# kjyv/FloBaRoID

Measured on AMD Instinct MI355X. Metric: regressor samples/s (fused regressor->Gram pass) + TSQR TFLOP/s, WALK-MAN 31-DOF float-base, higher is better.
Workload: dtype f64

## Files before the change

### flobaroid_amd/csrc/fbr_gram64.h

```cpp
#pragma once
#define FBR_G64_SWZ(c) (2 * ((c) & 15))
#include <algorithm>
#include <type_traits>
#include <utility>

#include "fbr_kinid.h"

struct FbrGram64Tile {
    int col[FBR_TILE];
    std::vector<int> path;
    int friction = 0;
    int lo = 0, hi = 0;
};

struct FbrGram64 {
    int NT = 0;
    int NF = 0;
    int nlev = 0, fb = 0, flev = 0, ntr = 0, maxact = 0, npw = 0, wpb = 8;
    long blk_doubles = 0;
    std::vector<int> trow;
    std::vector<int> slab;
    int nstage = 0, base_stages = 0;
    std::vector<int> stage_lev;
    std::vector<int> lev_begin;
// ... 356 lines not shown
                                    int tiling = 1)
{
    if (gp.T != 1 || (gp.k > 0 && gp.rhs_tiles)) return false;
    std::vector<FbrGram64Tile> prog;
    if (!fbr_gram64_program_tiles(hm, gp, prog)) return false;
    std::vector<int> pairs;
    for (size_t s = 0; s < gp.slots.size(); s++) {
        const int pi = gp.slots[s].pair;
        if (pi < 0) continue;
        if (gp.pairs[pi].mode != 0) return false;
        pairs.insert(pairs.end(), {gp.pairs[pi].I, gp.pairs[pi].J});
    }
    bool ok = fbr_gram64_build_tiles(hm, gp.cfg, prog, pairs, g, force_tiles, wide16) && fbr_gram64_lds_bytes(g) <= FBR_G64_LDS_MAX;
    g.tiling = 0;
    if (!ok || !tiling) return ok;
    std::vector<FbrGram64Tile> fill;
    fbr_gram64_fill_tiles(hm, prog, fill);
    FbrGram64 c;
    if (fbr_gram64_build_tiles(hm, gp.cfg, fill, {}, c, force_tiles, wide16) && fbr_gram64_lds_bytes(c) <= FBR_G64_LDS_MAX &&
        (c.mfma_per_block < g.mfma_per_block || (c.mfma_per_block == g.mfma_per_block && c.ntr < g.ntr))) {
        g = std::move(c);
        g.tiling = 1;
    }
    return true;
}

#define FBR_G64_WORDS 18
#define FBR_G64_FRIC 4
struct FbrGram64Producer {
    int nparts = 1, nslots = 1, step0[FBR_KINWRITE_PARTS] = {0, 0, 0, 0}, nsteps[FBR_KINWRITE_PARTS] = {0, 0, 0, 0};
    std::vector<long long> rel;
    std::vector<int> lcol;
    std::vector<int> steps;
};

static inline bool fbr_gram64_build_producer(const FbrHostModel &hm, const FbrGram64 &g, FbrGram64Producer &pr)
{
    std::vector<int> tile_of(hm.cols, -1), slot_of(hm.cols, -1);
    for (int t = 0; t < g.NT; t++)
        for (int sl = 0; sl < FBR_TILE; sl++)
            if (g.tiles[t].col[sl] >= 0 && g.tiles[t].col[sl] < hm.cols) {
                tile_of[g.tiles[t].col[sl]] = t;
                slot_of[g.tiles[t].col[sl]] = sl;
            }
    std::vector<double> lcost(hm.L, 30.0);
    for (int c = 0; c < hm.ninert; c++)
        if (tile_of[c] >= 0) lcost[hm.coldesc[c].link] += 10.0 + (double)(hm.fb + hm.path[hm.coldesc[c].link].size());
    std::vector<FbrKinIdProgram> progs;
    std::vector<std::vector<char>> own;
    try {
        fbr_kinid_build_parts(hm, lcost, FBR_KINWRITE_PARTS, progs, own);
    } catch (const std::exception &) {
        return false;
    }
    pr.nparts = (int)progs.size();
    pr.rel.assign((size_t)pr.nparts * FBR_G64_WORDS * hm.L, 0);
    pr.lcol.assign((size_t)pr.nparts * (10 + FBR_G64_FRIC) * hm.L, -1);
    const int nfric = hm.n > 0 ? (hm.cols - hm.ninert) / hm.n : 0;
    if (nfric > FBR_G64_FRIC) return false;
    auto word = [](long long tile_row, int sl) { return ((tile_row * 1024 + sl * 32) * 8) | (long long)FBR_G64_SWZ(sl) | (1LL << 62); };
    for (int c = 0; c < hm.ninert; c++) {
        const int t = tile_of[c], sl = slot_of[c], l = hm.coldesc[c].link, pidx = hm.coldesc[c].pidx;
        if (t < 0) continue;
        if (!FbrGramProgram::nested(g.tiles[t].path, hm.path[l]) || hm.path[l].size() > g.tiles[t].path.size()) return false;
        const long long tr0 = (long long)g.trow[(size_t)t * g.nlev + g.tile_lo[t]] - g.tile_lo[t];
        if (tr0 < 0) return false;
        for (int pq = 0; pq < pr.nparts; pq++)
            if (own[pq][l]) {
                long long *w14 = &pr.rel[((size_t)pq * hm.L + l) * FBR_G64_WORDS];
                w14[pidx] = word(tr0, sl);
                if (g.fcol_tile[c] >= 0) {
                    if (pidx >= 4) return false;
                    w14[10 + pidx] = word(g.trow[(size_t)g.fcol_tile[c] * g.nlev], g.fcol_slot[c]);
                }
                pr.lcol[((size_t)pq * hm.L + l) * 10 + pidx] = c;
            }
    }
    for (int c = hm.ninert; c < hm.cols; c++) {
        const int t = tile_of[c], sl = slot_of[c], d = hm.coldesc[c].joint, p = (c - hm.ninert) / std::max(hm.n, 1);
        if (t < 0) continue;
        int l = -1;
        for (int x = 0; x < hm.L; x++)
            if (hm.dof[x] == d) l = x;
        if (l < 0 || p >= FBR_G64_FRIC || hm.path[l].empty() || hm.path[l].back() != d) return false;
        const int lv = hm.fb + (int)hm.path[l].size() - 1;
        if (lv < g.tile_lo[t] || g.trow[(size_t)t * g.nlev + lv] < 0) return false;
        const long long tr0 = (long long)g.trow[(size_t)t * g.nlev + g.tile_lo[t]] - g.tile_lo[t];
        if (tr0 < 0) return false;
        for (int pq = 0; pq < pr.nparts; pq++)
            if (own[pq][l]) {
                pr.rel[((size_t)pq * hm.L + l) * FBR_G64_WORDS + 14 + p] = word(tr0, sl);
                pr.lcol[(size_t)pr.nparts * 10 * hm.L + ((size_t)pq * hm.L + l) * FBR_G64_FRIC + p] = c;
            }
    }
    pr.steps.clear();
    pr.nslots = 1;
    for (int pq = 0; pq < pr.nparts; pq++) {
        pr.step0[pq] = (int)(pr.steps.size() / FBR_KINID_STEP);
        pr.nsteps[pq] = progs[pq].nsteps;
        pr.nslots = std::max(pr.nslots, progs[pq].nslots);
        pr.steps.insert(pr.steps.end(), progs[pq].steps.begin(), progs[pq].steps.begin() + (size_t)progs[pq].nsteps * FBR_KINID_STEP);
    }
    return true;
}

static inline bool fbr_gram64_build_producer(const FbrHostModel &hm, const FbrGramProgram &, const FbrGram64 &g, FbrGram64Producer &pr)
{
    return fbr_gram64_build_producer(hm, g, pr);
}

#define FBR_G64_MAXK 2
#include "fbr_mom_lanes.h"
FBR_HD int fbr_gram64_mom_count(int cols, int k) { return k * cols + k * (k + 1) / 2; }
FBR_HD void fbr_gram64_mom_target(int cols, int k, int idx, int *row, int *col)
{
    if (idx < k * cols) {
        *row = idx % cols;
        *col = cols + idx / cols;
        return;
    }
    int e = idx - k * cols, i = 0;
    while (e >= k - i) e -= k - i, i++;
    *row = cols + i;
    *col = cols + i + e;
}

#define FBR_G64_LANECOL_RHS 24
static inline std::vector<int> fbr_gram64_lane_columns(const FbrGram64Producer &pr, int L)
{
    std::vector<int> t((size_t)pr.nparts * L * 64, -1);
    for (int pq = 0; pq < pr.nparts; pq++)
        for (int l = 0; l < L; l++)
            for (int r = 0; r < FBR_G64_MAXK; r++) {
                int *row = &t[((size_t)pq * L + l) * 64];
                for (int p = 0; p < 10; p++) {
                    const int c = pr.lcol[((size_t)pq * L + l) * 10 + p];
// ... 122 lines not shown
        const int ls = min(lane, valid - 1);
        const long s = base + ls;
        const bool live = lane < valid;
        const double *mysq = sq + ls * ldn, *mysdq = sdq + ls * ldn, *mysddq = sddq + ls * ldn, *myw = sw + ls * ldw, *myt = st + ls * ldw;
        const long slot_off = blk * blk_doubles + (long)(lane >> 5) * 512;
        const int s31 = lane & 31;
        auto state = [&](int d, double &a, double &b, double &c) {
            a = mysq[d];
            b = mysdq[d];
            c = mysddq[d];
        };
        auto basest = [&](double *v6, double *a6, double *e3) {
            for (int i = 0; i < 6; i++) {
                v6[i] = bv[s * 6 + i];
                a6[i] = ba[s * 6 + i];
            }
            for (int i = 0; i < 3; i++) e3[i] = rpy[s * 3 + i];
        };
        auto save = [&](int b, int i, double v) { scr[(b * FBR_LINK_REC + i) * 64] = v; };
        auto load = [&](int b, int i) { return scr[(b * FBR_LINK_REC + i) * 64]; };
        auto consts = [&](int l, double *rR, double *rp, double *ax) {
            const fbr_cdouble_ptr cR = (fbr_cdouble_ptr)(unsigned long)m.restR, cp = (fbr_cdouble_ptr)(unsigned long)m.restp,
                                  ca = (fbr_cdouble_ptr)(unsigned long)m.axis;
            for (int i = 0; i < 9; i++) rR[i] = cR[9 * l + i];
            for (int i = 0; i < 3; i++) {
                rp[i] = cp[3 * l + i];
                ax[i] = ca[3 * l + i];
            }
        };
        const unsigned vlane = (unsigned)(((unsigned long)slot_off + (unsigned long)s31) << 3);
        auto link = [&](int l, int depth, const double *rec, const double (*Sst)[6], const int *lvd, double *F) {
            (void)F;
            if (wr.base_only) depth = 0;
            int mycol = -1;
            if (domom) mycol = glcol[l * 64];
            __builtin_amdgcn_s_waitcnt(0x0F70);
            double macc = 0.0;
            auto mom_sum = [&](auto g0c, auto ngc, auto p0c, auto nqc, const double *v, int r) {
                constexpr int G0 = decltype(g0c)::value, NG = decltype(ngc)::value, P0 = decltype(p0c)::value, NQ = decltype(nqc)::value;
                double u[NG];
#pragma unroll
                for (int i = 0; i < NG; i++) u[i] = (G0 + i >= P0 && G0 + i < P0 + NQ) ? v[G0 + i - P0] : 0.0;
                const double sum = fbr_mom_lanes_sum<NG>(u, live, mx);
                if (G0 == 0 ? (lane & 15) == 6 * r : (lane & 7) == 1 + 6 * r) macc += sum;
            };
            long d10[10], dF[4];
#pragma unroll
            for (int pp = 0; pp < 10; pp++) d10[pp] = cdst[((long)part * m.L + l) * FBR_G64_WORDS + pp];
#pragma unroll
            for (int pp = 0; pp < 4; pp++) dF[pp] = cdst[((long)part * m.L + l) * FBR_G64_WORDS + 10 + pp];
            auto ft_of = [&](int ro, double *F) {
#pragma unroll
                for (int i = 0; i < 6; i++)
                    if (i < m.fb) F[i] = myt[ro + i];
#pragma unroll
                for (int j = 0; j < MAXD; j++)
                    if (j < depth) {
                        const double tj = myt[ro + m.fb + lvd[j]];
#pragma unroll
                        for (int i = 0; i < 6; i++) F[i] += Sst[j][i] * tj;
                    }
            };
            double Ft[6] = {0.0, 0.0, 0.0, 0.0, 0.0, 0.0};
            if constexpr (KR == 1) {
                if (wr.k) {
#pragma unroll
// ... 422 lines not shown
```

### flobaroid_amd/csrc/fbr_gram_api.hip

```cpp
#define FBR_KERNELS_GRAM
#include "fbr_internal.h"

static int get_deal(GramHolder *h, int wpg, GramHolder::Deal *out, bool base_only = false)
{
    const int key = wpg | (base_only ? 1 << 24 : 0);
    auto it = h->deals.find(key);
    if (it != h->deals.end()) {
        *out = it->second;
        return FBR_OK;
    }
    const std::vector<int> n = fbr_gram_deal(h->prog, wpg, base_only);
    std::vector<int2> tab;
    std::vector<int> begin(h->prog.T + 1, 0), given(h->prog.T, 0);
    for (int p = 0; p < h->prog.T; p++) begin[p + 1] = begin[p] + n[p];
    while ((int)tab.size() < begin[h->prog.T])
        for (int p = 0; p < h->prog.T; p++)
            if (given[p] < n[p]) tab.push_back(make_int2(p, given[p]++ | (n[p] << 16)));
    GramHolder::Deal d;
    int rc;
    if ((rc = upload(h->pool, tab, &d.tab))) return rc;
    if ((rc = upload(h->pool, begin, &d.begin))) return rc;
    h->deals[key] = d;
    *out = d;
    return FBR_OK;
// ... 227 lines not shown
{
    const int Pa = m->hm.cols + k;
    const size_t cnt = (size_t)Pa * Pa;
    int rc;
    if ((rc = m->gram_r_tmp.ensure(cnt * sizeof(double)))) return rc;
    double *R = m->gram_r_tmp.as<double>();
    if ((rc = tsqr_impl(m, st, nullptr, 0, rhs, k, w, nullptr, R, FBR_DEVICE, nullptr))) return rc;
    double *G = G_out;
    if (out_mem == FBR_HOST) {
        if ((rc = m->g_tmp.ensure(cnt * sizeof(double)))) return rc;
        G = m->g_tmp.as<double>();
        if (accumulate) HIPCHK(hipMemcpyAsync(G, G_out, cnt * sizeof(double), hipMemcpyHostToDevice, m->stream));
    }
    hipLaunchKernelGGL(fbr_rtr_kernel, dim3(1024), dim3(256), 0, m->stream, Pa, R, G, accumulate ? 1 : 0);
    HIPCHK(hipGetLastError());
    return finish_output(m, G, G_out, cnt, out_mem);
}
static size_t gram64_plds(const FbrHostModel &hm, int k, bool has_w)
{
    return ((size_t)3 * 64 * (std::max(hm.n, 1) | 1) + (size_t)((has_w ? 1 : 0) + k) * 64 * (hm.rows | 1)) * sizeof(double);
}

static int get_gram64(fbr_model *m, GramHolder *h)
{
    if (h->g64_state) return FBR_OK;
    h->g64_state = -1;
    const FbrHostModel &hm = m->hm;
    if (m->kinid.nsteps <= 0 || !fbr_gram64_build(hm, h->prog, h->g64, m->opt.gram_force_tiles != 0, m->opt.gram_lane_waves >= 16,
                                                         (int)m->opt.gram_lane_tiling))
        return FBR_OK;
    FbrGram64 &g = h->g64;
    if (fbr_gram64_lds_bytes(g) > FBR_G64_LDS_MAX) return FBR_OK;
    if (gram64_plds(hm, h->prog.k, true) > 160 * 1024) return FBR_OK;
    if (!fbr_gram64_build_producer(hm, g, h->g64p)) return FBR_OK;
    std::vector<int> wgbegin{0, 0};
    int rc;
    if ((rc = upload(h->pool, g.slab, &h->d64_slab)) || (rc = upload(h->pool, g.lev_begin, &h->d64_levb)) || (rc = upload(h->pool, g.pieces, &h->d64_pieces)) ||
        (rc = upload(h->pool, g.wmeta, &h->d64_wmeta)) || (rc = upload(h->pool, h->g64p.lcol, &h->d64_lcol)) ||
        (rc = upload(h->pool, fbr_gram64_lane_columns(h->g64p, hm.L), &h->d64_lanecol)) ||
        (rc = upload(h->pool, h->g64p.steps, &h->d64_steps)) ||
        (rc = upload(h->pool, g.slot_tiles, &h->d64_slot_tiles)) || (rc = upload(h->pool, g.tilecol, &h->d64_tilecol)) ||
        (rc = upload(h->pool, g.stage_lev, &h->d64_stagelev)) || (!g.runs.empty() && (rc = upload(h->pool, g.runs, &h->d64_runs))))
        return rc;
    h->g64_state = 1;
    return FBR_OK;
}

static int gram64_serves(fbr_model *m, GramHolder *h, int k, bool *serves)
{
    *serves = false;
    if (!m->opt.gram_lane || k > FBR_G64_MAXK || (k > 0 && !h->moments)) return FBR_OK;
    if (int rc = get_gram64(m, h)) return rc;
    *serves = h->g64_state == 1;
    return FBR_OK;
}

static long gram64_chunk_blocks(const FbrGram64 &g) { return std::max<long>(1, (long)((size_t)3 * 1024 * 1024 * 1024 / ((size_t)g.blk_doubles * 8))); }

static int gram64_wg_table(GramHolder *h, int wgs, const int **out)
{
    auto it = h->d64_wb.find(wgs);
    if (it == h->d64_wb.end()) {
        std::vector<int> wb{0, wgs};
        const int *dwb = nullptr;
        if (int rc = upload(h->pool, wb, &dwb)) return rc;
        it = h->d64_wb.emplace(wgs, dwb).first;
    }
    *out = it->second;
    return FBR_OK;
}

static int gram64_ensure_images(fbr_model *m, GramHolder *h, long chb)
{
// ... 27 lines not shown
static int gram64_setup(fbr_model *m, GramHolder *h, bool base_only, Gram64Launch *L)
{
    const FbrGram64 &g = h->g64;
    L->kp = kinid_params(m, 0, h->g64p.nslots, h->d64_steps);
    L->pgrid_max = kinimg_by_depth(m, [](auto D) { return D <= 10 ? 2 : 1; }) * m->num_cus;
    if (int rc = h->scr64.ensure((size_t)L->pgrid_max * h->g64p.nparts * std::max(h->g64p.nslots, 1) * FBR_LINK_REC * 64 * sizeof(double))) return rc;
    DevGram64 &dg = L->dg;
    dg.NT = g.NT + g.NF;
    dg.nlev = g.nlev;
    dg.maxact = g.maxact;
    dg.npieces = (int)g.pieces.size() / 2;
    dg.blk_doubles = g.blk_doubles;
    dg.slab = h->d64_slab;
    dg.lev_begin = h->d64_levb;
    dg.pieces = h->d64_pieces;
    dg.wmeta = h->d64_wmeta;
    dg.nstage = base_only ? g.base_stages : g.nstage;
    dg.stage_lev = h->d64_stagelev;
    dg.runs = g.runs.empty() ? nullptr : h->d64_runs;
    L->gk = g.wpb == 16 ? fbr_gram64_kernel<10, 16>
            : g.npw == 10   ? fbr_gram64_kernel<10, 8>
            : g.runs.empty() ? fbr_gram64_kernel<FBR_ONE_SEGW * FBR_ONE_NSEG, 8> : fbr_gram64_kernel<FBR_ONE_SEGW * FBR_ONE_NSEG, 8, true>;
    L->glds = fbr_gram64_lds_bytes(g);
    L->vnpw = g.npw * (g.wpb / 8);
    HIPCHK(hipFuncSetAttribute((const void *)L->gk, hipFuncAttributeMaxDynamicSharedMemorySize, (int)L->glds));
    return FBR_OK;
}

static DevKinWrite gram64_kinwrite(const fbr_model *m, const GramHolder *h, int b, int k, bool has_w, bool base_only, long group_samples)
{
    DevKinWrite kw{};
    kw.lcol10 = h->d64_lcol;
    kw.lanecol = h->d64_lanecol;
    kw.dst = (const long *)h->dst64[b].p;
    kw.ninert = m->hm.ninert;
    kw.cols = m->hm.cols;
    kw.k = k;
    kw.has_w = has_w ? 1 : 0;
    kw.flev = h->g64.flev;
    kw.base_only = base_only ? 1 : 0;
    kw.group_samples = group_samples;
    kw.nparts = h->g64p.nparts;
    for (int pq = 0; pq < FBR_KINWRITE_PARTS; pq++) {
        kw.part_nsteps[pq] = h->g64p.nsteps[pq];
        kw.part_step0[pq] = h->g64p.step0[pq];
    }
    return kw;
}

static int gram64_produce(fbr_model *m, GramHolder *h, const Gram64Launch &L, const DevKinWrite &kw, int pblocks, size_t plds, long cs,
                          const DevStates &d, long so, const double *rhs, int k, const double *w, double *mom)
{
    const FbrHostModel &hm = m->hm;
    return kinimg_by_depth(m, [&](auto D) -> int {
        const auto kernel = k == 2 ? (kw.has_w ? fbr_kinimg_kernel<D, true, 2> : fbr_kinimg_kernel<D, false, 2>)
                                   : (kw.has_w ? fbr_kinimg_kernel<D, true> : fbr_kinimg_kernel<D, false>);
        HIPCHK(hipFuncSetAttribute((const void *)kernel, hipFuncAttributeMaxDynamicSharedMemorySize, (int)plds));
        hipLaunchKernelGGL(kernel, dim3(pblocks), dim3(64 * h->g64p.nparts), plds, m->stream, m->dm, L.kp, kw, cs, h->g64.blk_doubles, d.q + so * hm.n,
                           d.dq + so * hm.n, d.ddq + so * hm.n, d.bv ? d.bv + so * 6 : nullptr, d.ba ? d.ba + so * 6 : nullptr,
                           d.rpy ? d.rpy + so * 3 : nullptr, rhs ? rhs + (size_t)so * hm.rows * k : nullptr, w ? w + (size_t)so * hm.rows : nullptr,
                           h->scr64.as<double>(), mom, d.sign ? d.sign + so * hm.n : nullptr);
        HIPCHK(hipGetLastError());
        return FBR_OK;
    });
}

// ... 36 lines not shown
{
    const FbrHostModel &hm = m->hm;
    double *p = m->st_chunk[b].as<double>();
    auto put = [&](const double *src, size_t per, const double **dst) -> int {
        *dst = nullptr;
        if (!src || per == 0) return FBR_OK;
        HIPCHK(hipMemcpyAsync(p, src + (size_t)s0 * per, (size_t)cs * per * sizeof(double), hipMemcpyHostToDevice, cps));
        *dst = p;
        p += (size_t)cs * per;
        return FBR_OK;
    };
    *dc = d;
    int rc;
    if ((rc = put(d.q, hm.n, &dc->q)) || (rc = put(d.dq, hm.n, &dc->dq)) || (rc = put(d.ddq, hm.n, &dc->ddq)) || (rc = put(d.bv, 6, &dc->bv)) ||
        (rc = put(d.ba, 6, &dc->ba)) || (rc = put(d.rpy, 3, &dc->rpy)) || (rc = put(d.sign, hm.n, &dc->sign)) ||
        (rc = put(rhs, (size_t)hm.rows * k, crhs)) || (rc = put(w, hm.rows, cw)))
        return rc;
    return FBR_OK;
}

static int gram64_pass(fbr_model *m, GramHolder *h, const DevStates &d, const double *drhs, const double *dw, int k, double *G, bool base_only,
                       bool h2d_chunked)
{
    const FbrHostModel &hm = m->hm;
    const FbrGram64 &g = h->g64;
    const long S = d.S;
    int rc;
    const long nblocks = (S + 63) / 64;
    long chb = gram64_chunk_blocks(g);
    if (h2d_chunked) chb = std::min<long>(chb, 7L * m->num_cus);
    if (m->opt.chunk_samples >= 1) chb = std::min(gram64_chunk_blocks(g), std::max<long>(1, ((long)m->opt.chunk_samples + 63) / 64));
    chb = std::min(nblocks, chb);
    if (chb < nblocks && chb > m->num_cus) chb = chb / m->num_cus * m->num_cus;
    long chs = chb * 64;
    if (m->opt.chunk_samples >= 1) chs = std::min(chs, (long)m->opt.chunk_samples);
    if ((rc = gram64_ensure_images(m, h, chb))) return rc;
    Gram64Launch L;
    if ((rc = gram64_setup(m, h, base_only, &L))) return rc;
    const size_t plds = gram64_plds(hm, k, dw != nullptr);
    const int pblocks = (int)std::min<long>(chb, (long)L.pgrid_max);
    const int gwgs = (int)std::min<long>(chb, (long)m->num_cus);
    if (k) {
        if ((rc = h->mom64.ensure((size_t)L.pgrid_max * fbr_gram64_mom_count(hm.cols, k) * sizeof(double)))) return rc;
        HIPCHK(hipMemsetAsync(h->mom64.p, 0, (size_t)pblocks * fbr_gram64_mom_count(hm.cols, k) * sizeof(double), m->stream));
    }
    if ((rc = m->partial.ensure((size_t)m->num_cus * g.wpb * g.npw * 256 * sizeof(double)))) return rc;
    int launches = 0, first_wgs = 0;
    if (h2d_chunked) {
        if ((rc = ensure_stage_buffers(m, d, k, dw, chs, 2)) || (rc = ensure_copy_stream(m))) return rc;
        HIPCHK(hipEventRecord(m->ev_fork, m->stream));
    }
    struct Staged {
        DevStates dc;
        long o;
        const double *rhs, *w;
    };
    auto stage = [&](long c, Staged &out) -> int {
        const long s0 = c * chs, cs = std::min(chs, S - s0);
        const int b = (int)(c & 1);
        out = {d, s0, drhs, dw};
        if (!h2d_chunked) return FBR_OK;
        HIPCHK(hipStreamWaitEvent(m->copy, m->ev_pack_rec[b] ? m->ev_pack[b] : m->ev_fork, 0));
        ProfScope ps(m, FBR_PROF_H2D, m->copy);
        if (int r3 = stage_chunk(m, d, drhs, k, dw, s0, cs, b, m->copy, &out.dc, &out.rhs, &out.w)) return r3;
        out.o = 0;
        HIPCHK(hipEventRecord(m->ev_h2d[b], m->copy));
        return FBR_OK;
    };
    Staged cur, nxt;
    if (S > 0 && (rc = stage(0, nxt))) return rc;
    for (long s0 = 0; s0 < S; s0 += chs, launches++) {
        const long cs = std::min(chs, S - s0), nb = (cs + 63) / 64;
        const int b = launches & 1;
        cur = nxt;
        if (s0 + chs < S && (rc = stage(launches + 1, nxt))) return rc;
        if (h2d_chunked) HIPCHK(hipStreamWaitEvent(m->stream, m->ev_h2d[b], 0));
        {
            ProfScope ps(m, FBR_PROF_PACK);
            if ((rc = gram64_produce(m, h, L, gram64_kinwrite(m, h, b, k, dw != nullptr, base_only, 0), pblocks, plds, cs, cur.dc, cur.o, cur.rhs, k,
                                     cur.w, k ? h->mom64.as<double>() : nullptr)))
                return rc;
            if (cs & 63) {
                hipLaunchKernelGGL(fbr_gram64_tail_zero_kernel, dim3(16, 1), dim3(256), 0, m->stream, h->img64[b].as<double>(), g.blk_doubles, nb, g.ntr, (int)(cs & 63));
                HIPCHK(hipGetLastError());
            }
            if (h2d_chunked) {
                HIPCHK(hipEventRecord(m->ev_pack[b], m->stream));
                m->ev_pack_rec[b] = true;
            }
        }
        const int wgs = (int)std::min<long>(nb, (long)gwgs);
        if (launches == 0) first_wgs = wgs;
        if (wgs > first_wgs) {
            set_err("internal: Gram launch wider than the first one of the call");
            return FBR_E_INVALID;
        }
        {
            ProfScope ps(m, FBR_PROF_GRAM);
            hipLaunchKernelGGL(L.gk, dim3(first_wgs), dim3(g.wpb * 64), L.glds, m->stream, L.dg, nb, h->img64[b].as<double>(), m->partial.as<double>(),
                               launches > 0 ? 1 : 0);
            HIPCHK(hipGetLastError());
        }
    }
    if (launches > 0) {
        ProfScope ps(m, FBR_PROF_REDUCE);
        const int *wgb = nullptr;
        if ((rc = gram64_wg_table(h, first_wgs, &wgb)) || (rc = gram64_reduce(m, h, L, first_wgs, wgb, 1, G))) return rc;
        if (k) {
// ... 434 lines not shown
```

### flobaroid_amd/csrc/fbr_internal.h

```cpp
#pragma once
#include <hip/hip_runtime.h>
#include <unistd.h>

#include <algorithm>
#include <cstdint>
#include <cstdio>
#include <cstdlib>
#include <cstring>
#include <map>
#include <memory>
#include <numeric>
#include <string>
#include <vector>

#include "../../include/fbr.h"
#include "fbr_options.h"
#include "fbr_kernels.h"
#include "fbr_kinid.h"
#include "fbr_capsule.h"
#include "fbr_capsule_grad.h"
#include "fbr_gram64.h"
#include "fbr_tsqr_work.h"
#include "fbr_weights.h"

// ... 51 lines not shown
        if (p) (void)hipFree(p);
        p = nullptr;
        bytes = 0;
    }
    template <class T> T *as() { return (T *)p; }
};

template <class T> static inline int upload(std::vector<DevBuf> &pool, const std::vector<T> &v, const T **out)
{
    pool.emplace_back();
    DevBuf &b = pool.back();
    size_t n = std::max<size_t>(v.size(), 1) * sizeof(T);
    int rc = b.ensure(n);
    if (rc) return rc;
    if (!v.empty()) HIPCHK(hipMemcpy(b.p, v.data(), v.size() * sizeof(T), hipMemcpyHostToDevice));
    *out = (const T *)b.p;
    return FBR_OK;
}

struct GramHolder {
    FbrGramProgram prog;
    DevGram dev;
    std::vector<DevBuf> pool;
    DevBuf pimg[2];
    bool moments = false;
    DevBuf mom[2];
    bool mom_clean[2] = {false, false};
    const int *itemcol = nullptr;
    size_t lds_bytes = 0;
    size_t pack_lds_bytes = 0;
    int g64_state = 0;
    FbrGram64 g64;
    FbrGram64Producer g64p;
    const int *d64_slab = nullptr, *d64_levb = nullptr, *d64_pieces = nullptr, *d64_wmeta = nullptr, *d64_lcol = nullptr, *d64_lanecol = nullptr,
              *d64_steps = nullptr, *d64_slot_tiles = nullptr, *d64_tilecol = nullptr, *d64_stagelev = nullptr,
              *d64_runs = nullptr;
    DevBuf img64[2], dst64[2], mom64, scr64;
    long img64_blocks = 0;
    std::map<int, const int *> d64_wb;
    struct Deal { const int2 *tab; const int *begin; };
    std::map<int, Deal> deals;
};

struct fbr_model {
    FbrOptions opt;
    FbrHostModel hm;
    DevModel dm;
    int device = 0;
    pid_t pid = 0;
    int num_cus = 256;
    hipStream_t own_stream = nullptr, stream = nullptr;
    hipStream_t side = nullptr;
    hipStream_t copy = nullptr;
    hipEvent_t ev_pack[2] = {nullptr, nullptr}, ev_gram[2] = {nullptr, nullptr}, ev_fork = nullptr, ev_h2d[2] = {nullptr, nullptr};
    hipEvent_t ev_done[2] = {nullptr, nullptr};
    int64_t next_ticket = 0;
    int64_t waited_ticket = -1;
    bool submitting = false;
    bool ev_gram_rec[2] = {false, false};
    bool ev_pack_rec[2] = {false, false};
    DevBuf rec2;
    std::vector<DevBuf> tables;
    std::map<int, std::unique_ptr<GramHolder>> gram;
    DevBuf st_q, st_dq, st_ddq, st_bv, st_ba, st_rpy, st_sign, st_aux, st_aux2, st_x;
    DevBuf rec, partial, out_tmp, g_tmp;
    DevBuf st_chunk[2];
    DevBuf fd[7];
// ... 160 lines not shown
```

### flobaroid_amd/csrc/fbr_kinid.h

```cpp
#pragma once
#include <type_traits>
#include <vector>

#include "fbr_math.h"
#include "fbr_program.h"

#define FBR_KINID_STEP 8
#define FBR_KINID_MAXD 24

#define FBR_KINWRITE_PARTS 4

template <int D, int... Ds, class F> inline auto fbr_by_depth(int maxlvl, F &&f)
{
    if constexpr (sizeof...(Ds) > 0)
        if (maxlvl > D) return fbr_by_depth<Ds...>(maxlvl, f);
    return f(std::integral_constant<int, D>());
}

#if defined(__HIPCC__)
typedef const __attribute__((address_space(4))) long *fbr_clong_ptr;
typedef const __attribute__((address_space(4))) int *fbr_cint_ptr;
typedef const __attribute__((address_space(4))) double *fbr_cdouble_ptr;
#endif

// ... 49 lines not shown
    }
    const int nslots = (int)holder.size();
    p.nslots = nslots;
    p.maxlvl = maxlvl;
    p.endflush.assign(std::max(maxlvl, 1), -1);
    for (int v = 0; v < maxlvl; v++) p.endflush[v] = lvldof[v];
}

static inline void fbr_kinid_build_parts(const FbrHostModel &hm, const std::vector<double> &cost, int nparts, std::vector<FbrKinIdProgram> &progs,
                                         std::vector<std::vector<char>> &own)
{
    nparts = std::max(1, std::min(nparts, hm.L));
    double total = 0.0;
    for (int l = 0; l < hm.L; l++) total += cost[l];
    progs.assign(nparts, FbrKinIdProgram());
    own.assign(nparts, std::vector<char>(hm.L, 0));
    double acc = 0.0;
    int part = 0;
    for (int k = 0; k < hm.L; k++) {
        const int l = hm.order[k];
        if (part + 1 < nparts && acc >= total * (part + 1) / nparts && hm.L - k >= nparts - part - 1) part++;
        own[part][l] = 1;
        acc += cost[l];
    }
    for (int p = 0; p < nparts; p++) {
        std::vector<char> keep = own[p];
        for (int l = 0; l < hm.L; l++)
            if (own[p][l])
                for (int a = hm.parent[l]; a >= 0 && !keep[a]; a = hm.parent[a]) keep[a] = 1;
        fbr_kinid_build(hm, progs[p], &keep);
    }
}

#if defined(__HIPCC__) && defined(__HIP_DEVICE_COMPILE__)
#define FBR_UNI(x) __builtin_amdgcn_readfirstlane(x)
#else
#define FBR_UNI(x) (x)
#endif

template <int MAXD, bool ACC, class StateFn, class BaseFn, class SlotSave, class SlotLoad, class LinkFn, class EmitFn, class ConstFn>
FBR_HD void fbr_kinid_lane(int nsteps, int maxlvl, const int *steps, const int *endflush, int floating, const double *g, int fb,
                           StateFn state, BaseFn basest, SlotSave save, SlotLoad load, LinkFn link, EmitFn emit, ConstFn consts)
{
    double P[FBR_LINK_REC];
    double Sst[MAXD][6], tac[MAXD];
    int lvd[MAXD];
    double T[6] = {0, 0, 0, 0, 0, 0};
#if defined(__HIPCC__)
#pragma unroll
#endif
    for (int j = 0; j < MAXD; j++) {
        tac[j] = 0.0;
        lvd[j] = 0;
        for (int i = 0; i < 6; i++) Sst[j][i] = 0.0;
    }
    for (int k = 0; k < nsteps; k++) {
#if defined(__HIP_DEVICE_COMPILE__)
        const fbr_cint_ptr st = (fbr_cint_ptr)(unsigned long)(steps + k * FBR_KINID_STEP);
#else
        const int *st = steps + k * FBR_KINID_STEP;
#endif
        const int l = FBR_UNI(st[0]), psrc = FBR_UNI(st[1]), psave = FBR_UNI(st[2]), jt = FBR_UNI(st[3]), d = FBR_UNI(st[4]), lvl = FBR_UNI(st[5]),
                  depth = FBR_UNI(st[6]), fd = FBR_UNI(st[7]);
        double out[FBR_LINK_REC], Sv[6] = {0, 0, 0, 0, 0, 0};
        if (psrc < 0) {
            double v6[6] = {0, 0, 0, 0, 0, 0}, a6[6] = {0, 0, 0, 0, 0, 0}, e3[3] = {0, 0, 0};
// ... 70 lines not shown
}

#if defined(__HIPCC__)
struct DevKinId {
    int nsteps, maxlvl, nslots, ldn;
    const int *steps, *endflush;
};
struct DevKinExt {
    long T, tiles, nblk;
    double *val;
    long *idx;
};
FBR_HD double fbr_ext_value(int k, double v)
{
    if (k == 2) return fabs(v);
    if (k == 3) return v != v ? 0.0 : fmin(fabs(v), 1.7976931348623157e308);
    return v;
}
FBR_HD bool fbr_ext_take(int k, double a, double b)
{
    if (b != b) return false;
    return a != a || (k == 0 ? a < b : a > b);
}
typedef __attribute__((address_space(1))) char *fbr_gchar_ptr;
typedef __attribute__((address_space(1))) double *fbr_gdouble_ptr;
struct DevKinWrite {
    const int *lcol10, *colrec;
    const int *lanecol = nullptr;
    const long *dst;
    int ninert, cols, k, has_w;
    int flev;
    int base_only;
    long group_samples;
    int nparts, part_nsteps[FBR_KINWRITE_PARTS], part_step0[FBR_KINWRITE_PARTS];
};
#endif

#if defined(__HIPCC__) && defined(FBR_KERNELS_CORE)

template <int MAXD, bool EXT = false>
__global__ __launch_bounds__(64) void fbr_kinid_kernel(DevModel m, DevKinId p, long S, const double *__restrict__ q, const double *__restrict__ dq,
                                                       const double *__restrict__ ddq, const double *__restrict__ bv,
                                                       const double *__restrict__ ba, const double *__restrict__ rpy,
                                                       const double *__restrict__ sign, const double *__restrict__ vel_sign,
                                                       const double *__restrict__ x, int mode, double *__restrict__ tau, double *__restrict__ scratch, int flink, double fpx,
                                                       double fpy, double fpz, DevKinExt ex)
{
    extern __shared__ __attribute__((aligned(16))) double smem[];
    const int lane = threadIdx.x, n = m.n, ldn = p.ldn;
    double *sq = smem, *sdq = sq + 64 * ldn, *sddq = sdq + 64 * ldn;
    double *scr = scratch + (long)blockIdx.x * p.nslots * FBR_LINK_REC * 64 + lane;
    const long nblk = EXT ? ex.nblk : (S + 63) >> 6;
    for (long blk = blockIdx.x; blk < nblk; blk += gridDim.x) {
        long base, i0 = 0;
        int valid;
        if constexpr (EXT) {
            const long c = blk / ex.tiles;
            i0 = (blk - c * ex.tiles) << 6;
            base = c * ex.T + i0;
            valid = (int)min(64L, ex.T - i0);
        } else {
            base = blk << 6;
            valid = (int)min(64L, S - base);
        }
        __syncthreads();
        {
// ... 370 lines not shown
```

### flobaroid_amd/csrc/fbr_options.h

```cpp
#pragma once
#include <cstring>

struct FbrOptions {
    double link_merge = 1;
    double regroup = 1;
    double reduce_min_work = 1e9;
    double reduce_grouped_min_samples = 512;
    double chunk_samples = 0;
    double min_chunks = 4;
    double h2d_chunked = 1;
    double fused_id = 1;
    double gram_lane_waves = 8;
    double gram_force_tiles = 1;
    double gram_lane = 1;
    double gram_lane_tiling = 1;
    double gram_shape = 0;
    double gram_rhs_tile = 0;
    double gram_orient = 1;
    double gram_serial = 0;
    double gram_timing = 0;
    double tsqr_groups = 1;
    double tsqr_group_min_samples = 24000;
    double tsqr_reorder = 1;
    double tsqr_tree_one_wg = 0;
    double tsqr_narrow = 1;
    double tsqr_narrow_tall = 1;
    double tsqr_force_group = 1;
    double tsqr_lane_writer = 1;
    double tsqr_writer = 0;
    double tsqr_side_trees_beside = 0;
    double tsqr_prologue_overlap = 1;
    double tsqr_timing = 0;
    double tsqr_short_call_factors = 1;
};

struct FbrOptionKey {
    const char *name;
    double FbrOptions::*field;
    bool rebuild_programs;
};

static inline const FbrOptionKey *fbr_option_keys(int *count)
{
    static const FbrOptionKey keys[] = {
        {"link_merge", &FbrOptions::link_merge, false},
        {"regroup", &FbrOptions::regroup, false},
        {"reduce_min_work", &FbrOptions::reduce_min_work, false},
        {"reduce_grouped_min_samples", &FbrOptions::reduce_grouped_min_samples, false},
        {"chunk_samples", &FbrOptions::chunk_samples, false},
        {"min_chunks", &FbrOptions::min_chunks, false},
        {"h2d_chunked", &FbrOptions::h2d_chunked, false},
        {"fused_id", &FbrOptions::fused_id, false},
        {"gram_lane", &FbrOptions::gram_lane, false},
        {"gram_force_tiles", &FbrOptions::gram_force_tiles, true},
        {"gram_lane_waves", &FbrOptions::gram_lane_waves, true},
        {"gram_lane_tiling", &FbrOptions::gram_lane_tiling, true},
        {"gram_shape", &FbrOptions::gram_shape, true},
        {"gram_rhs_tile", &FbrOptions::gram_rhs_tile, true},
        {"gram_orient", &FbrOptions::gram_orient, true},
        {"gram_serial", &FbrOptions::gram_serial, false},
        {"gram_timing", &FbrOptions::gram_timing, false},
        {"tsqr_groups", &FbrOptions::tsqr_groups, false},
        {"tsqr_group_min_samples", &FbrOptions::tsqr_group_min_samples, false},
        {"tsqr_reorder", &FbrOptions::tsqr_reorder, false},
        {"tsqr_tree_one_wg", &FbrOptions::tsqr_tree_one_wg, false},
        {"tsqr_narrow", &FbrOptions::tsqr_narrow, false},
        {"tsqr_narrow_tall", &FbrOptions::tsqr_narrow_tall, false},
        {"tsqr_lane_writer", &FbrOptions::tsqr_lane_writer, false},
        {"tsqr_force_group", &FbrOptions::tsqr_force_group, false},
        {"tsqr_writer", &FbrOptions::tsqr_writer, false},
        {"tsqr_side_trees_beside", &FbrOptions::tsqr_side_trees_beside, false},
        {"tsqr_prologue_overlap", &FbrOptions::tsqr_prologue_overlap, false},
        {"tsqr_timing", &FbrOptions::tsqr_timing, false},
        {"tsqr_short_call_factors", &FbrOptions::tsqr_short_call_factors, false},
    };
    *count = (int)(sizeof(keys) / sizeof(keys[0]));
    return keys;
}

static inline const FbrOptionKey *fbr_option_find(const char *name)
{
    int n = 0;
    const FbrOptionKey *k = fbr_option_keys(&n);
    for (int i = 0; i < n; i++)
        if (name && !strcmp(k[i].name, name)) return &k[i];
    return nullptr;
}
```

Before: 88.08 million.

## Skip unowned links in producer, add optional partition rebalance and chunk-round planning

Builds a per-part, per-link 'none' table marking links whose destination words are all zero, uploads it, and makes the kinematic producer return early for such links by default. It also adds two options that are off by default: a cost-model search for better cut points when splitting the link order across four producer parts, and a chunk plan that picks chunk sizes to reduce GPU rounds. The default path skips the write/moment work for ancestor-only links, in exchange for one extra global load per link.

```diff
diff --git a/flobaroid_amd/csrc/fbr_gram64.h b/flobaroid_amd/csrc/fbr_gram64.h
--- a/flobaroid_amd/csrc/fbr_gram64.h
+++ b/flobaroid_amd/csrc/fbr_gram64.h
@@ -412,9 +412,86 @@
     std::vector<long long> rel;
     std::vector<int> lcol;
     std::vector<int> steps;
+    std::vector<int> none;
+    std::vector<int> starts;
 };
 
-static inline bool fbr_gram64_build_producer(const FbrHostModel &hm, const FbrGram64 &g, FbrGram64Producer &pr)
+struct FbrGram64PartModel {
+    double a = 300.0, b = 400.0, c = 5.0, d = 1.0;
+};
+struct FbrGram64PartStats {
+    int steps = 0, links = 0, entries = 0, unowned = 0, discarded = 0;
+    double cost = 0.0;
+};
+static inline std::vector<FbrGram64PartStats> fbr_gram64_part_stats(const FbrHostModel &hm, const std::vector<int> &ncol, const std::vector<int> &nfr,
+                                                                    const std::vector<int> &starts, int k, const FbrGram64PartModel &pm)
+{
+    std::vector<FbrGram64PartStats> st(starts.size() - 1);
+    for (size_t p = 0; p + 1 < starts.size(); p++) {
+        std::vector<char> keep(hm.L, 0), mine(hm.L, 0);
+        for (int i = starts[p]; i < starts[p + 1]; i++) {
+            const int l = hm.order[i];
+            mine[l] = 1;
+            for (int a = l; a >= 0 && !keep[a]; a = hm.parent[a]) keep[a] = 1;
+        }
+        for (int l = 0; l < hm.L; l++) {
+            if (!keep[l]) continue;
+            const int e = ncol[l] * (hm.fb + (int)hm.path[l].size()) + nfr[l];
+            st[p].steps++;
+            if (mine[l]) {
+                st[p].links++;
+                st[p].entries += e;
+            } else {
+                st[p].unowned++;
+                st[p].discarded += 10 * (hm.fb + (int)hm.path[l].size());
+            }
+        }
+        st[p].cost = pm.a * st[p].steps + pm.b * st[p].links + (pm.c + (k > 0 ? pm.d : 0.0)) * st[p].entries;
+    }
+    return st;
+}
+static inline std::vector<int> fbr_gram64_cut_parts(const FbrHostModel &hm, const std::vector<int> &ncol, const std::vector<int> &nfr,
+                                                    const std::vector<int> &old, int k, const FbrGram64PartModel &pm)
+{
+    const int L = hm.L, np = (int)old.size() - 1;
+    if (np != FBR_KINWRITE_PARTS || L > 256 || L < np) return old;
+    std::vector<double> rc((size_t)(L + 1) * (L + 1), 0.0);
+    const double ce = pm.c + (k > 0 ? pm.d : 0.0);
+    std::vector<char> keep(L);
+    for (int i = 0; i < L; i++) {
+        std::fill(keep.begin(), keep.end(), 0);
+        double cost = 0.0;
+        for (int j = i; j < L; j++) {
+            const int l = hm.order[j];
+            for (int a = l; a >= 0 && !keep[a]; a = hm.parent[a]) keep[a] = 1, cost += pm.a;
+            cost += pm.b + ce * (ncol[l] * (hm.fb + (int)hm.path[l].size()) + nfr[l]);
+            rc[(size_t)i * (L + 1) + j + 1] = cost;
+        }
+    }
+    auto R = [&](int i, int j) { return rc[(size_t)i * (L + 1) + j]; };
+    auto worst = [&](int c1, int c2, int c3) { return std::max(std::max(R(0, c1), R(c1, c2)), std::max(R(c2, c3), R(c3, L))); };
+    int best[3] = {old[1], old[2], old[3]}, bestdist = 0;
+    double bestmax = worst(old[1], old[2], old[3]);
+    for (int c1 = 1; c1 < L - 2; c1++) {
+        if (R(0, c1) > bestmax) break;
+        for (int c2 = c1 + 1; c2 < L - 1; c2++) {
+            if (R(c1, c2) > bestmax) break;
+            for (int c3 = c2 + 1; c3 < L; c3++) {
+                const double w = worst(c1, c2, c3);
+                const int dist = std::abs(c1 - old[1]) + std::abs(c2 - old[2]) + std::abs(c3 - old[3]);
+                if (w < bestmax || (w == bestmax && dist < bestdist)) {
+                    bestmax = w;
+                    bestdist = dist;
+                    best[0] = c1, best[1] = c2, best[2] = c3;
+                }
+            }
+        }
+    }
+    return {0, best[0], best[1], best[2], L};
+}
+
+static inline bool fbr_gram64_build_producer(const FbrHostModel &hm, const FbrGram64 &g, FbrGram64Producer &pr, int cut = 0, int k = 1,
+                                             const std::vector<int> *force_starts = nullptr)
 {
     std::vector<int> tile_of(hm.cols, -1), slot_of(hm.cols, -1);
     for (int t = 0; t < g.NT; t++)
@@ -430,6 +507,24 @@
     std::vector<std::vector<char>> own;
     try {
         fbr_kinid_build_parts(hm, lcost, FBR_KINWRITE_PARTS, progs, own);
+        pr.starts = fbr_kinid_parts_starts(hm, own);
+        if (cut || force_starts) {
+            std::vector<int> ncol(hm.L, 0), nfr(hm.L, 0);
+            for (int c = 0; c < hm.cols; c++) {
+                if (tile_of[c] < 0) continue;
+                if (c < hm.ninert) {
+                    ncol[hm.coldesc[c].link]++;
+                } else {
+                    for (int x = 0; x < hm.L; x++)
+                        if (hm.dof[x] == hm.coldesc[c].joint) nfr[x]++;
+                }
+            }
+            const std::vector<int> starts = force_starts ? *force_starts : fbr_gram64_cut_parts(hm, ncol, nfr, pr.starts, k, FbrGram64PartModel());
+            if (starts != pr.starts) {
+                fbr_kinid_build_parts_at(hm, starts, progs, own);
+                pr.starts = starts;
+            }
+        }
     } catch (const std::exception &) {
         return false;
     }
@@ -473,6 +568,11 @@
                 pr.lcol[(size_t)pr.nparts * 10 * hm.L + ((size_t)pq * hm.L + l) * FBR_G64_FRIC + p] = c;
             }
     }
+    pr.none.assign((size_t)pr.nparts * hm.L, 1);
+    for (int pq = 0; pq < pr.nparts; pq++)
+        for (int l = 0; l < hm.L; l++)
+            for (int i = 0; i < FBR_G64_WORDS; i++)
+                if (pr.rel[((size_t)pq * hm.L + l) * FBR_G64_WORDS + i]) pr.none[(size_t)pq * hm.L + l] = 0;
     pr.steps.clear();
     pr.nslots = 1;
     for (int pq = 0; pq < pr.nparts; pq++) {
@@ -482,6 +582,38 @@
         pr.steps.insert(pr.steps.end(), progs[pq].steps.begin(), progs[pq].steps.begin() + (size_t)progs[pq].nsteps * FBR_KINID_STEP);
     }
     return true;
+}
+
+struct FbrGram64ChunkPlan {
+    long chb = 0, last_cap = 0, chunks = 0, gram_rounds = 0, prod_rounds = 0;
+};
+static inline FbrGram64ChunkPlan fbr_gram64_chunk_plan(long nblocks, long cap, long num_cus, long pgrid_max, int rule)
+{
+    auto plan = [&](long chb, long last_cap) {
+        FbrGram64ChunkPlan p;
+        p.chb = chb;
+        p.last_cap = last_cap;
+        const long pb = std::min(chb, pgrid_max);
+        for (long left = nblocks; left > 0;) {
+            const long nb = left <= last_cap ? left : chb;
+            p.chunks++;
+            p.gram_rounds += (nb + num_cus - 1) / num_cus;
+            p.prod_rounds += (nb + pb - 1) / pb;
+            left -= nb;
+        }
+        return p;
+    };
+    const long a0 = cap / num_cus;
+    FbrGram64ChunkPlan best = plan(a0 * num_cus, a0 * num_cus);
+    if (!rule) return best;
+    for (long a = a0; a >= 1; a--) {
+        const FbrGram64ChunkPlan p = plan(a * num_cus, cap);
+        if (p.gram_rounds != best.gram_rounds ? p.gram_rounds < best.gram_rounds
+            : p.prod_rounds != best.prod_rounds ? p.prod_rounds < best.prod_rounds
+                                                : p.chunks < best.chunks)
+            best = p;
+    }
+    return best;
 }
 
 static inline bool fbr_gram64_build_producer(const FbrHostModel &hm, const FbrGramProgram &, const FbrGram64 &g, FbrGram64Producer &pr)
@@ -670,6 +802,7 @@
         auto link = [&](int l, int depth, const double *rec, const double (*Sst)[6], const int *lvd, double *F) {
             (void)F;
             if (wr.base_only) depth = 0;
+            if (wr.none && ((fbr_cint_ptr)(unsigned long)wr.none)[(long)part * m.L + l]) return;
             int mycol = -1;
             if (domom) mycol = glcol[l * 64];
             __builtin_amdgcn_s_waitcnt(0x0F70);
diff --git a/flobaroid_amd/csrc/fbr_gram_api.hip b/flobaroid_amd/csrc/fbr_gram_api.hip
--- a/flobaroid_amd/csrc/fbr_gram_api.hip
+++ b/flobaroid_amd/csrc/fbr_gram_api.hip
@@ -283,13 +283,13 @@
     FbrGram64 &g = h->g64;
     if (fbr_gram64_lds_bytes(g) > FBR_G64_LDS_MAX) return FBR_OK;
     if (gram64_plds(hm, h->prog.k, true) > 160 * 1024) return FBR_OK;
-    if (!fbr_gram64_build_producer(hm, g, h->g64p)) return FBR_OK;
+    if (!fbr_gram64_build_producer(hm, g, h->g64p, m->opt.gram_lane_parts_cut != 0, h->prog.k)) return FBR_OK;
     std::vector<int> wgbegin{0, 0};
     int rc;
     if ((rc = upload(h->pool, g.slab, &h->d64_slab)) || (rc = upload(h->pool, g.lev_begin, &h->d64_levb)) || (rc = upload(h->pool, g.pieces, &h->d64_pieces)) ||
         (rc = upload(h->pool, g.wmeta, &h->d64_wmeta)) || (rc = upload(h->pool, h->g64p.lcol, &h->d64_lcol)) ||
         (rc = upload(h->pool, fbr_gram64_lane_columns(h->g64p, hm.L), &h->d64_lanecol)) ||
-        (rc = upload(h->pool, h->g64p.steps, &h->d64_steps)) ||
+        (rc = upload(h->pool, h->g64p.steps, &h->d64_steps)) || (rc = upload(h->pool, h->g64p.none, &h->d64_none)) ||
         (rc = upload(h->pool, g.slot_tiles, &h->d64_slot_tiles)) || (rc = upload(h->pool, g.tilecol, &h->d64_tilecol)) ||
         (rc = upload(h->pool, g.stage_lev, &h->d64_stagelev)) || (!g.runs.empty() && (rc = upload(h->pool, g.runs, &h->d64_runs))))
         return rc;
@@ -383,6 +383,7 @@
     DevKinWrite kw{};
     kw.lcol10 = h->d64_lcol;
     kw.lanecol = h->d64_lanecol;
+    kw.none = m->opt.gram_lane_skip_unowned != 0 ? h->d64_none : nullptr;
     kw.dst = (const long *)h->dst64[b].p;
     kw.ninert = m->hm.ninert;
     kw.cols = m->hm.cols;
@@ -485,11 +486,19 @@
     if (m->opt.chunk_samples >= 1) chb = std::min(gram64_chunk_blocks(g), std::max<long>(1, ((long)m->opt.chunk_samples + 63) / 64));
     chb = std::min(nblocks, chb);
     if (chb < nblocks && chb > m->num_cus) chb = chb / m->num_cus * m->num_cus;
+    Gram64Launch L;
+    if ((rc = gram64_setup(m, h, base_only, &L))) return rc;
+    long last_blocks = 0;
+    if (m->opt.gram_lane_chunk_rounds != 0 && !h2d_chunked && m->opt.chunk_samples < 1 && chb < nblocks && chb >= m->num_cus) {
+        const FbrGram64ChunkPlan cp = fbr_gram64_chunk_plan(nblocks, gram64_chunk_blocks(g), m->num_cus, L.pgrid_max, 1);
+        chb = cp.chb;
+        last_blocks = cp.last_cap;
+    }
     long chs = chb * 64;
     if (m->opt.chunk_samples >= 1) chs = std::min(chs, (long)m->opt.chunk_samples);
-    if ((rc = gram64_ensure_images(m, h, chb))) return rc;
-    Gram64Launch L;
-    if ((rc = gram64_setup(m, h, base_only, &L))) return rc;
+    const long last_s = last_blocks > 0 ? last_blocks * 64 : chs;
+    auto chunk_len = [&](long s0) { return S - s0 <= last_s ? S - s0 : chs; };
+    if ((rc = gram64_ensure_images(m, h, std::min(nblocks, std::max(chb, last_blocks))))) return rc;
     const size_t plds = gram64_plds(hm, k, dw != nullptr);
     const int pblocks = (int)std::min<long>(chb, (long)L.pgrid_max);
     const int gwgs = (int)std::min<long>(chb, (long)m->num_cus);
@@ -509,7 +518,7 @@
         const double *rhs, *w;
     };
     auto stage = [&](long c, Staged &out) -> int {
-        const long s0 = c * chs, cs = std::min(chs, S - s0);
+        const long s0 = c * chs, cs = chunk_len(s0);
         const int b = (int)(c & 1);
         out = {d, s0, drhs, dw};
         if (!h2d_chunked) return FBR_OK;
@@ -522,11 +531,12 @@
     };
     Staged cur, nxt;
     if (S > 0 && (rc = stage(0, nxt))) return rc;
-    for (long s0 = 0; s0 < S; s0 += chs, launches++) {
-        const long cs = std::min(chs, S - s0), nb = (cs + 63) / 64;
+    for (long s0 = 0, cs = 0; s0 < S; s0 += cs, launches++) {
+        cs = chunk_len(s0);
+        const long nb = (cs + 63) / 64;
         const int b = launches & 1;
         cur = nxt;
-        if (s0 + chs < S && (rc = stage(launches + 1, nxt))) return rc;
+        if (s0 + cs < S && (rc = stage(launches + 1, nxt))) return rc;
         if (h2d_chunked) HIPCHK(hipStreamWaitEvent(m->stream, m->ev_h2d[b], 0));
         {
             ProfScope ps(m, FBR_PROF_PACK);
diff --git a/flobaroid_amd/csrc/fbr_internal.h b/flobaroid_amd/csrc/fbr_internal.h
--- a/flobaroid_amd/csrc/fbr_internal.h
+++ b/flobaroid_amd/csrc/fbr_internal.h
@@ -107,7 +107,7 @@
     int g64_state = 0;
     FbrGram64 g64;
     FbrGram64Producer g64p;
-    const int *d64_slab = nullptr, *d64_levb = nullptr, *d64_pieces = nullptr, *d64_wmeta = nullptr, *d64_lcol = nullptr, *d64_lanecol = nullptr,
+    const int *d64_slab = nullptr, *d64_levb = nullptr, *d64_pieces = nullptr, *d64_wmeta = nullptr, *d64_lcol = nullptr, *d64_lanecol = nullptr, *d64_none = nullptr,
               *d64_steps = nullptr, *d64_slot_tiles = nullptr, *d64_tilecol = nullptr, *d64_stagelev = nullptr,
               *d64_runs = nullptr;
     DevBuf img64[2], dst64[2], mom64, scr64;
diff --git a/flobaroid_amd/csrc/fbr_kinid.h b/flobaroid_amd/csrc/fbr_kinid.h
--- a/flobaroid_amd/csrc/fbr_kinid.h
+++ b/flobaroid_amd/csrc/fbr_kinid.h
@@ -105,6 +105,34 @@
     }
 }
 
+static inline void fbr_kinid_build_parts_at(const FbrHostModel &hm, const std::vector<int> &starts, std::vector<FbrKinIdProgram> &progs,
+                                            std::vector<std::vector<char>> &own)
+{
+    const int nparts = (int)starts.size() - 1;
+    if (nparts < 1 || starts[0] != 0 || starts[nparts] != hm.L) throw std::runtime_error("fbr_kinid_build_parts_at: cut points outside the order");
+    progs.assign(nparts, FbrKinIdProgram());
+    own.assign(nparts, std::vector<char>(hm.L, 0));
+    for (int p = 0; p < nparts; p++) {
+        if (starts[p + 1] < starts[p]) throw std::runtime_error("fbr_kinid_build_parts_at: cut points out of order");
+        for (int k = starts[p]; k < starts[p + 1]; k++) own[p][hm.order[k]] = 1;
+        std::vector<char> keep = own[p];
+        for (int l = 0; l < hm.L; l++)
+            if (own[p][l])
+                for (int a = hm.parent[l]; a >= 0 && !keep[a]; a = hm.parent[a]) keep[a] = 1;
+        fbr_kinid_build(hm, progs[p], &keep);
+    }
+}
+static inline std::vector<int> fbr_kinid_parts_starts(const FbrHostModel &hm, const std::vector<std::vector<char>> &own)
+{
+    std::vector<int> starts{0};
+    for (size_t p = 0; p < own.size(); p++) {
+        int cnt = 0;
+        for (int l = 0; l < hm.L; l++) cnt += own[p][l] != 0;
+        starts.push_back(starts.back() + cnt);
+    }
+    return starts;
+}
+
 #if defined(__HIPCC__) && defined(__HIP_DEVICE_COMPILE__)
 #define FBR_UNI(x) __builtin_amdgcn_readfirstlane(x)
 #else
@@ -241,6 +269,7 @@
     int flev;
     int base_only;
     long group_samples;
+    const int *none = nullptr;
     int nparts, part_nsteps[FBR_KINWRITE_PARTS], part_step0[FBR_KINWRITE_PARTS];
 };
 #endif
diff --git a/flobaroid_amd/csrc/fbr_options.h b/flobaroid_amd/csrc/fbr_options.h
--- a/flobaroid_amd/csrc/fbr_options.h
+++ b/flobaroid_amd/csrc/fbr_options.h
@@ -14,6 +14,9 @@
     double gram_force_tiles = 1;
     double gram_lane = 1;
     double gram_lane_tiling = 1;
+    double gram_lane_skip_unowned = 1;
+    double gram_lane_parts_cut = 0;
+    double gram_lane_chunk_rounds = 0;
     double gram_shape = 0;
     double gram_rhs_tile = 0;
     double gram_orient = 1;
@@ -55,6 +58,9 @@
         {"gram_force_tiles", &FbrOptions::gram_force_tiles, true},
         {"gram_lane_waves", &FbrOptions::gram_lane_waves, true},
         {"gram_lane_tiling", &FbrOptions::gram_lane_tiling, true},
+        {"gram_lane_skip_unowned", &FbrOptions::gram_lane_skip_unowned, true},
+        {"gram_lane_parts_cut", &FbrOptions::gram_lane_parts_cut, true},
+        {"gram_lane_chunk_rounds", &FbrOptions::gram_lane_chunk_rounds, true},
         {"gram_shape", &FbrOptions::gram_shape, true},
         {"gram_rhs_tile", &FbrOptions::gram_rhs_tile, true},
         {"gram_orient", &FbrOptions::gram_orient, true},
```

Result: faster. 90.05 million, median of 6 (+2.2%).
